# kontera-technologies/redis-bloomfilter

Hardware: AMD Instinct MI355X
Metric: keys/sec (insert, include?) per GPU and whole node; % of HBM random-access roofline (higher is better)
Workload: dtype u32

## Files before the change

redis-bloomfilter_amd/csrc/bf_binned.hip:

```cpp
#include "bf_device.h"

#include <algorithm>
#include <cmath>
#include <cstdlib>

using namespace bfdev;

namespace {
__device__ __forceinline__ void stage_store(uint32_t* p, uint32_t v) { __builtin_nontemporal_store(v, p); }
}

namespace {

constexpr int kTile = 1024;
constexpr int kStageVec = 16384 / 16;
constexpr uint32_t kMaxSup = 256;
constexpr uint32_t kMaxOwners = 256;
constexpr uint32_t kChunkBuckets = 512;
constexpr uint32_t kMaxRel = 9;
constexpr uint32_t kMaxBlocks = 512;
constexpr uint32_t kMaxFrontBlocks = 16384;
constexpr uint32_t kGroupBlocks = 64;
constexpr uint32_t kTileProbes = 12288;
constexpr int kSlots = 12;
constexpr int kWideSlots = 16;
constexpr uint32_t kTwoKeys = 6;
constexpr uint32_t kMaxTilesPerBlock = 16;
constexpr uint32_t kBlockProbes = 8192;
constexpr int kChunkPerLane = kBlockProbes / kTile;
constexpr uint32_t kRunsPerPass = 1024;
constexpr uint32_t kMidBuckets = 128;
constexpr uint32_t kMidParts = 2;
constexpr uint32_t kApplyLanes = 1024;
constexpr uint32_t kPipeLanes = 1024;

__device__ __forceinline__ uint32_t block_excl_scan(uint32_t v, uint32_t* s_w, uint32_t* total) {
    const uint32_t lane = threadIdx.x & 63u, wid = threadIdx.x >> 6, nw = blockDim.x >> 6;
    const uint32_t x = wave_incl_scan(v);
    if (lane == 63u) s_w[wid] = x;
    __syncthreads();
    if (wid == 0) {
        const uint32_t s = wave_incl_scan(lane < nw ? s_w[lane] : 0u);
        if (lane < nw) s_w[lane] = s;
    }
    __syncthreads();
    const uint32_t r = (wid ? s_w[wid - 1] : 0u) + x - v;
    if (total) *total = s_w[nw - 1];
    __syncthreads();
    return r;
}

template <bool KEYS, int SLOTS, bool DIG = false>
__device__ __forceinline__ void bin_front_body(BfGeom g, const uint8_t* __restrict__ keys16,
                                                          const uint64_t* __restrict__ offsets, uint64_t bias,
                                                          uint64_t n, uint32_t tile_keys, uint32_t tiles_per_block,
                                                          uint32_t sup_log2, uint32_t nsup,
                                                          uint32_t* __restrict__ level1,
                                                          uint32_t* __restrict__ level1_key,
                                                          uint16_t* __restrict__ stab, uint32_t* __restrict__ gcnt,
                                                          uint8_t* __restrict__ out8) {
    __shared__ uint64_t s_off[kTile + 1];
    __shared__ uint4 s_stage[kStageVec + kStageSlackVec];
    __shared__ uint32_t s_cnt[kMaxSup], s_lbase[kMaxSup], s_gcnt[kMaxSup];
    __shared__ uint32_t s_w[16];
    __shared__ uint32_t s_sorted[kTile * SLOTS];
    __shared__ uint32_t s_key[KEYS ? kTile * SLOTS : 1];
    const uint32_t t = threadIdx.x;
    if (t < kMaxSup) {
        s_cnt[t] = 0;
        s_gcnt[t] = 0;
    }
    __syncthreads();
    const uint32_t k = g.k;
    const uint32_t kpl = tile_keys / kTile;
    const uint64_t smask = (1ull << sup_log2) - 1ull;
    const uint64_t ntiles = (n + tile_keys - 1) / tile_keys;
    const uint64_t tb0 = (uint64_t)blockIdx.x * tiles_per_block;
    const uint64_t tb1 = (tb0 + tiles_per_block < ntiles) ? tb0 + tiles_per_block : ntiles;
    for (uint64_t tile = tb0; tile < tb1; ++tile) {
        const uint64_t key0 = tile * tile_keys;
        const uint32_t tk = (uint32_t)((n - key0) < (uint64_t)tile_keys ? (n - key0) : tile_keys);
        uint4 H0 = make_uint4(0, 0, 0, 0), H1 = make_uint4(0, 0, 0, 0);
        if constexpr (DIG) {
            const uint4* dig = reinterpret_cast<const uint4*>(keys16);
            if (t < tk) H0 = dig[key0 + t];
            if (kTile + t < tk) H1 = dig[key0 + kTile + t];
        } else {
            for_key_tile<kTile, kStageVec>(keys16, offsets, bias, key0, tk < (uint32_t)kTile ? tk : kTile, s_off,
                                           s_stage, g.key_status, [&](auto staged, uint32_t, const uint32_t* src, uint32_t s, uint32_t L) {
                uint32_t H[5];
                sha1_any<decltype(staged)::value>(src, s, L, H);
                H0 = make_uint4(H[0], H[1], H[2], H[3]);
            });
            if (tk > (uint32_t)kTile) {
                for_key_tile<kTile, kStageVec>(keys16, offsets, bias, key0 + kTile, tk - kTile, s_off, s_stage,
                    g.key_status, [&](auto staged, uint32_t, const uint32_t* src, uint32_t s, uint32_t L) {
                        uint32_t H[5];
                        sha1_any<decltype(staged)::value>(src, s, L, H);
                        H1 = make_uint4(H[0], H[1], H[2], H[3]);
                    });
            }
        }
        const bool live0 = t < tk;
        const bool live1 = kpl == 2 && kTile + t < tk;
        if constexpr (KEYS) {
            if (live0) out8[key0 + t] = 1;
            if (live1) out8[key0 + kTile + t] = 1;
        }
        uint32_t tag[SLOTS], loc[SLOTS];
#pragma unroll
        for (int q = 0; q < SLOTS; ++q) {
            const bool second = kpl == 2 && q >= (int)kTwoKeys;
            const uint32_t i = second ? (uint32_t)q - kTwoKeys : (uint32_t)q;
            const bool live = i < k && (second ? live1 : live0);
            tag[q] = 0xFFFFFFFFu;
            loc[q] = 0;
            if (live) {
                const uint4 H = second ? H1 : H0;
                const uint64_t o = probe_offset(g, H.x, H.y, H.z, H.w, i);
                const uint32_t sb = (uint32_t)(o >> sup_log2);
                tag[q] = (sb << 16) | atomicAdd(s_cnt + sb, 1u);
                loc[q] = (uint32_t)(o & smask);
            }
        }
        __syncthreads();
        const uint32_t c = t < kMaxSup ? s_cnt[t] : 0u;
        const uint32_t ex = block_excl_scan(c, s_w, nullptr);
        if (t <= nsup) stab[(uint64_t)t * ntiles + tile] = (uint16_t)ex;
        if (t < kMaxSup) {
            s_lbase[t] = ex;
            s_gcnt[t] += c;
            s_cnt[t] = 0;
        }
        __syncthreads();
#pragma unroll
        for (int q = 0; q < SLOTS; ++q) {
            if (tag[q] != 0xFFFFFFFFu) {
                const uint32_t d = s_lbase[tag[q] >> 16] + (tag[q] & 0xFFFFu);
                s_sorted[d] = loc[q];
                if constexpr (KEYS) {
                    const bool second = kpl == 2 && q >= (int)kTwoKeys;
                    s_key[d] = (uint32_t)(key0 + (second ? kTile + t : t));
                }
            }
        }
        __syncthreads();
        const uint64_t seg = key0 * k;
        const uint32_t tp = tk * k;
        for (uint32_t j = t; j < tp; j += kTile) {
            stage_store(level1 + seg + j, s_sorted[j]);
            if constexpr (KEYS) level1_key[seg + j] = s_key[j];
        }
    }
    if (t < nsup) gcnt[(uint64_t)blockIdx.x * nsup + t] = s_gcnt[t];
}

template <bool DIG>
__global__ __launch_bounds__(kTile) __attribute__((amdgpu_waves_per_eu(8, 8)))
void bin_front_kernel(BfGeom g, const uint8_t* __restrict__ keys16, const uint64_t* __restrict__ offsets,
                      uint64_t bias, uint64_t n, uint32_t tile_keys, uint32_t tiles_per_block, uint32_t sup_log2,
                      uint32_t nsup, uint32_t* __restrict__ level1, uint32_t* __restrict__ level1_key,
                      uint16_t* __restrict__ stab, uint32_t* __restrict__ gcnt, uint8_t* __restrict__ out8) {
    bin_front_body<false, kSlots, DIG>(g, keys16, offsets, bias, n, tile_keys, tiles_per_block, sup_log2, nsup,
                                       level1, level1_key, stab, gcnt, out8);
}

template <bool KEYS, bool DIG = false>
__global__ __launch_bounds__(kTile) void bin_front_wide_kernel(BfGeom g, const uint8_t* __restrict__ keys16,
                                                               const uint64_t* __restrict__ offsets, uint64_t bias,
                                                               uint64_t n, uint32_t tile_keys,
                                                               uint32_t tiles_per_block, uint32_t sup_log2,
                                                               uint32_t nsup, uint32_t* __restrict__ level1,
                                                               uint32_t* __restrict__ level1_key,
                                                               uint16_t* __restrict__ stab, uint32_t* __restrict__ gcnt,
                                                               uint8_t* __restrict__ out8) {
    bin_front_body<KEYS, kWideSlots, DIG>(g, keys16, offsets, bias, n, tile_keys, tiles_per_block, sup_log2, nsup,
                                          level1, level1_key, stab, gcnt, out8);
}

__global__ __launch_bounds__(kTile) __attribute__((amdgpu_waves_per_eu(8, 8)))
void bin_front_wide_dig_kernel(BfGeom g, const uint8_t* __restrict__ keys16, const uint64_t* __restrict__ offsets,
                               uint64_t bias, uint64_t n, uint32_t tile_keys, uint32_t tiles_per_block,
                               uint32_t sup_log2, uint32_t nsup, uint32_t* __restrict__ level1,
                               uint32_t* __restrict__ level1_key, uint16_t* __restrict__ stab,
                               uint32_t* __restrict__ gcnt, uint8_t* __restrict__ out8) {
    bin_front_body<false, kWideSlots, true>(g, keys16, offsets, bias, n, tile_keys, tiles_per_block, sup_log2, nsup,
                                            level1, level1_key, stab, gcnt, out8);
}

__global__ __launch_bounds__(kTile)
void bin_front_keys_kernel(BfGeom g, const uint8_t* __restrict__ keys16, const uint64_t* __restrict__ offsets,
                           uint64_t bias, uint64_t n, uint32_t tile_keys, uint32_t tiles_per_block, uint32_t sup_log2,
                           uint32_t nsup, uint32_t* __restrict__ level1, uint32_t* __restrict__ level1_key,
                           uint16_t* __restrict__ stab, uint32_t* __restrict__ gcnt, uint8_t* __restrict__ out8) {
    bin_front_body<true, kSlots>(g, keys16, offsets, bias, n, tile_keys, tiles_per_block, sup_log2, nsup, level1,
                                 level1_key, stab, gcnt, out8);
}

template <typename Off, bool KEYS>
__device__ __forceinline__ void bin_front_offsets_body(const Off* __restrict__ local, uint64_t count,
                                                       uint32_t tiles_per_block, uint32_t sup_log2, uint32_t nsup,
                                                       uint32_t* __restrict__ level1,
                                                       uint32_t* __restrict__ level1_key,
                                                       uint16_t* __restrict__ stab, uint32_t* __restrict__ gcnt,
                                                       uint64_t bias, const unsigned long long* __restrict__ wcounts,
                                                       uint32_t wstride, uint64_t wcap, uint64_t limit,
                                                       uint8_t* __restrict__ oob_out) {
    __shared__ uint32_t s_cnt[kMaxSup], s_lbase[kMaxSup], s_gcnt[kMaxSup];
    __shared__ uint32_t s_w[16];
    __shared__ uint32_t s_sorted[kTileProbes];
    __shared__ uint16_t s_key[KEYS ? kTileProbes : 1];
    const uint32_t t = threadIdx.x;
    if (t < kMaxSup) {
        s_cnt[t] = 0;
        s_gcnt[t] = 0;
    }
    __syncthreads();
    const uint64_t smask = (1ull << sup_log2) - 1ull;
    const uint64_t ntiles = (count + kTileProbes - 1) / kTileProbes;
    const bool vec_ok = (reinterpret_cast<uintptr_t>(local) & 15u) == 0;
    static_assert(kTileProbes == kTile * kSlots, "a tile is kSlots entries per lane");
    const uint64_t tb0 = (uint64_t)blockIdx.x * tiles_per_block;
    const uint64_t tb1 = (tb0 + tiles_per_block < ntiles) ? tb0 + tiles_per_block : ntiles;
    for (uint64_t tile = tb0; tile < tb1; ++tile) {
        const uint64_t p0 = tile * kTileProbes;
        uint32_t tp = (uint32_t)((count - p0) < (uint64_t)kTileProbes ? (count - p0) : kTileProbes);
        if (wcounts) {
            const uint64_t w = p0 / wcap, i0 = p0 - w * wcap;
            uint64_t live = wcounts[w * wstride];
            if (live > wcap) live = 0;
            tp = live > i0 ? (uint32_t)(live - i0 < (uint64_t)tp ? live - i0 : tp) : 0u;
        }
        uint32_t tag[kSlots], loc[kSlots];
        Off ent[kSlots];
        const uint32_t j0 = t * (uint32_t)kSlots;
        if (vec_ok && j0 + kSlots <= tp) {
            constexpr int kNV = kSlots * (int)sizeof(Off) / 16;
            const uint4* src = reinterpret_cast<const uint4*>(local + p0 + j0);
            uint4 vb[kNV];
#pragma unroll
            for (int v = 0; v < kNV; ++v) vb[v] = src[v];
            __builtin_memcpy(ent, vb, sizeof(ent));
        } else {
#pragma unroll
            for (int q = 0; q < kSlots; ++q) ent[q] = j0 + q < tp ? local[p0 + j0 + q] : (Off)0;
        }
#pragma unroll
        for (int q = 0; q < kSlots; ++q) {
            const uint32_t j = j0 + (uint32_t)q;
            tag[q] = 0xFFFFFFFFu;
            loc[q] = 0;
            if (j < tp) {
                const uint64_t o = (uint64_t)ent[q] + bias;
                if (o < limit) {
                    const uint32_t sb = (uint32_t)(o >> sup_log2);
                    tag[q] = (sb << 16) | atomicAdd(s_cnt + sb, 1u);
                    loc[q] = (uint32_t)(o & smask);
                } else if (oob_out) {
                    oob_out[p0 + j] = 0;
                }
            }
        }
        __syncthreads();
        const uint32_t c = t < kMaxSup ? s_cnt[t] : 0u;
        const uint32_t ex = block_excl_scan(c, s_w, nullptr);
        if (t <= nsup) stab[(uint64_t)t * ntiles + tile] = (uint16_t)ex;
        if (t < kMaxSup) {
            s_lbase[t] = ex;
            s_gcnt[t] += c;
            s_cnt[t] = 0;
        }
        __syncthreads();
#pragma unroll
        for (int q = 0; q < kSlots; ++q)
            if (tag[q] != 0xFFFFFFFFu) {
                const uint32_t d = s_lbase[tag[q] >> 16] + (tag[q] & 0xFFFFu);
                s_sorted[d] = loc[q];
                if constexpr (KEYS) s_key[d] = (uint16_t)(t * (uint32_t)kSlots + (uint32_t)q);
            }
        __syncthreads();
        for (uint32_t j = t; j < tp; j += kTile) {
            level1[p0 + j] = s_sorted[j];
            if constexpr (KEYS) level1_key[p0 + j] = (uint32_t)p0 + s_key[j];
        }
    }
    if (t < nsup) gcnt[(uint64_t)blockIdx.x * nsup + t] = s_gcnt[t];
}

template <typename Off>
__global__ __launch_bounds__(kTile) __attribute__((amdgpu_waves_per_eu(8, 8)))
void bin_front_offsets_kernel(const Off* __restrict__ local, uint64_t count, uint32_t tiles_per_block,
                              uint32_t sup_log2, uint32_t nsup, uint32_t* __restrict__ level1,
                              uint16_t* __restrict__ stab, uint32_t* __restrict__ gcnt, uint64_t bias,
                              const unsigned long long* __restrict__ wcounts, uint32_t wstride, uint64_t wcap,
                              uint64_t limit) {
    bin_front_offsets_body<Off, false>(local, count, tiles_per_block, sup_log2, nsup, level1, nullptr, stab, gcnt,
                                       bias, wcounts, wstride, wcap, limit, nullptr);
}

template <typename Off>
__global__ __launch_bounds__(kTile) __attribute__((amdgpu_waves_per_eu(8, 8)))
void bin_front_offsets_keys_kernel(const Off* __restrict__ local, uint64_t count,
                                                                       uint32_t tiles_per_block, uint32_t sup_log2,
                                                                       uint32_t nsup, uint32_t* __restrict__ level1,
                                                                       uint32_t* __restrict__ level1_key,
                                                                       uint16_t* __restrict__ stab,
                                                                       uint32_t* __restrict__ gcnt, uint64_t bias,
                                                                       const unsigned long long* __restrict__ wcounts,
                                                                       uint32_t wstride, uint64_t wcap, uint64_t limit,
                                                                       uint8_t* __restrict__ out8) {
    bin_front_offsets_body<Off, true>(local, count, tiles_per_block, sup_log2, nsup, level1, level1_key, stab, gcnt,
                                      bias, wcounts, wstride, wcap, limit, out8);
}

__global__ __launch_bounds__(kMaxBlocks) void bin_group_sum_kernel(const uint32_t* __restrict__ gcnt,
                                                                   uint32_t nblocks, uint32_t nsup, uint32_t nq,
                                                                   uint32_t* __restrict__ gsum) {
    const uint32_t sb = blockIdx.x;
    for (uint32_t w = threadIdx.x; w < nq * kGroupBlocks; w += kMaxBlocks) {
        uint32_t v = w < nblocks ? gcnt[(uint64_t)w * nsup + sb] : 0u;
#pragma unroll
        for (int off = 32; off > 0; off >>= 1) v += (uint32_t)__shfl_xor((int)v, off);
        if ((w & 63u) == 0) gsum[sb * nq + w / kGroupBlocks] = v;
    }
}

constexpr uint32_t kScanPer = 4;
constexpr uint32_t kScanWindows = 1024 * kScanPer;
constexpr uint32_t kLocalScanPer = 4;
constexpr uint32_t kMaxGroups = 1024 * kLocalScanPer;
constexpr uint32_t kMaxWindows = kMaxSup * kMaxGroups;
__global__ __launch_bounds__(1024) void bin_group_scan_kernel(const uint32_t* __restrict__ gsum, uint32_t N,
                                                              uint32_t* __restrict__ base,
                                                              uint32_t* __restrict__ cb_base,
                                                              uint32_t* __restrict__ cb_window,
                                                              uint32_t* __restrict__ cb_start, uint32_t nq,
                                                              unsigned long long* __restrict__ totals) {
    __shared__ uint32_t s_w[16];
    __shared__ uint32_t s_cb[kScanWindows + 1];
    const uint32_t t = threadIdx.x;
    uint32_t v[kScanPer], cv[kScanPer], sum = 0, csum = 0;
#pragma unroll
    for (uint32_t e = 0; e < kScanPer; ++e) {
        const uint32_t w = kScanPer * t + e;
        v[e] = w < N ? gsum[w] : 0u;
        cv[e] = (v[e] + kBlockProbes - 1) / kBlockProbes;
        sum += v[e];
        csum += cv[e];
    }
    uint32_t total, ctotal;
    uint32_t ex = block_excl_scan(sum, s_w, &total);
    uint32_t cex = block_excl_scan(csum, s_w, &ctotal);
// ... 271 lines not shown
                if constexpr (CHUNK)
                    reinterpret_cast<uint32_t*>(cg.dir + (uint64_t)t * cg.dir_bytes)[tile] =
                        (gb + oc <= wcap) ? (uint32_t)gb : 0xFFFFFFFFu;
            }
            if constexpr (CHUNK) {
                const uint32_t S1 = cg.S + 1u;
                for (uint32_t e = t; e < P * S1; e += kTile) {
                    const uint32_t w = e / S1, sb = e - w * S1;
                    const uint32_t b0 = (w * cg.S) << sub_log2, b1 = (w * cg.S + sb) << sub_log2;
                    const uint32_t v = (b1 < NB ? s_lbase[b1] : tk * k) - s_lbase[b0];
                    reinterpret_cast<uint16_t*>(cg.dir + (uint64_t)w * cg.dir_bytes + 4 * cg.tiles)
                        [(uint64_t)sb * cg.tiles + tile] = (uint16_t)v;
                }
            }
        }
#pragma unroll
        for (int q = 0; q < SLOTS; ++q) {
            if (tag[q] != 0xFFFFFFFFu) {
                const uint32_t d = s_lbase[tag[q] >> 16] + (tag[q] & 0xFFFFu);
                s_lo[d] = lo[q];
                if constexpr (WIDE) s_hi[d] = hi[q];
                if constexpr (SLOT) {
                    const bool second = kpl == 2 && q >= (int)kTwoKeys;
                    s_key[d] = (uint16_t)(second ? kTile + t : t);
                }
            }
        }
        __syncthreads();
        const uint64_t seg = key0 * k;
        const uint32_t tp = tk * k;
        if constexpr (WIN) {
            uint32_t o = run_of(s_obase, P, t < tp ? t : 0u);
            for (uint32_t j = t; j < tp; j += kTile) {
                while (o + 1u < P && s_obase[o + 1u] <= j) ++o;
                const unsigned long long gb = s_gbase[o];
                if (gb != ~0ull) {
                    const uint64_t d = gb + (j - s_obase[o]);
                    static_cast<uint32_t*>(wsend)[d] = s_lo[j];
                    if constexpr (SLOT) {
                        if constexpr (CHUNK) reinterpret_cast<uint16_t*>(wslot)[d] = s_key[j];
                        else wslot[d] = (uint32_t)key0 + s_key[j];
                    }
                }
            }
            __syncthreads();
        } else {
            for (uint32_t j = t; j < tp; j += kTile) {
                lo1[seg + j] = s_lo[j];
                if constexpr (WIDE) hi1[seg + j] = s_hi[j];
                if constexpr (SLOT) key1[seg + j] = (uint32_t)key0 + s_key[j];
            }
            if constexpr (SLOT) __syncthreads();
        }
    }
    if constexpr (!WIN)
        if (t < P) gcnt[(uint64_t)blockIdx.x * P + t] = s_gcnt[t];
}

#define BF_ROUTE_FRONT_ARGS                                                                                     \
    BfGeom g, const uint8_t* __restrict__ keys16, const uint64_t* __restrict__ offsets, uint64_t bias, uint64_t n, \
        uint32_t tile_keys, uint32_t tiles_per_block, uint32_t P, uint32_t* __restrict__ lo1,                   \
        uint8_t* __restrict__ hi1, uint32_t* __restrict__ key1, uint16_t* __restrict__ stab,                     \
        uint32_t* __restrict__ gcnt, uint64_t wcap, unsigned long long* __restrict__ wcounts,                 \
        void* __restrict__ wsend, uint32_t* __restrict__ wslot, uint32_t nh
#define BF_ROUTE_FRONT_PASS \
    g, keys16, offsets, bias, n, tile_keys, tiles_per_block, P, lo1, hi1, key1, stab, gcnt, wcap, wcounts, wsend, wslot, nh
template <bool WIDE, bool SLOT, int SLOTS, bool WIN, bool CHUNK = false, bool DIG = false>
__global__ __launch_bounds__(kTile) void route_front_kernel(BF_ROUTE_FRONT_ARGS, BfChunks cg) {
    route_front_body<WIDE, SLOT, SLOTS, WIN, CHUNK, DIG>(BF_ROUTE_FRONT_PASS, cg);
}
template <bool SLOT, bool WIN, bool CHUNK = false, bool DIG = false>
__global__ __launch_bounds__(kTile) __attribute__((amdgpu_waves_per_eu(8, 8)))
void route_front32_kernel(BF_ROUTE_FRONT_ARGS, BfChunks cg) {
    route_front_body<false, SLOT, kSlots, WIN, CHUNK, DIG>(BF_ROUTE_FRONT_PASS, cg);
}
#undef BF_ROUTE_FRONT_PASS
#undef BF_ROUTE_FRONT_ARGS

template <bool SLOT, int SLOTS, bool HASH = false>
__global__ __launch_bounds__(kTile) __attribute__((amdgpu_waves_per_eu(8, 8)))
void route_chunks_idx_kernel(BfGeom g, const uint8_t* __restrict__ keys16, const uint64_t* __restrict__ offsets,
                             uint64_t bias, uint64_t n, uint32_t tile_keys,
                             uint32_t tiles_per_block, uint32_t P, uint64_t wcap,
                             unsigned long long* __restrict__ wcounts, uint32_t* __restrict__ wsend,
                             uint16_t* __restrict__ wslot, uint32_t nh, BfChunks cg) {
    static_assert(SLOTS <= 16 && kTile * SLOTS <= 65536, "a probe index is 4 bits, a sort slot 16");
    constexpr uint32_t NB = kChunkBuckets;
    constexpr uint32_t kOffVec = (8 * (kTile + 1) + 15) / 16;
    static_assert(!HASH || (SLOTS > kSlots && (kOffVec + kStageVec + kStageSlackVec) * 16 <= kTile * SLOTS * 2),
                  "the key stage fits the index buffer (one key per lane)");
    __shared__ uint4 s_idx4[kTile * SLOTS * 2 / 16];
    uint16_t* s_idx = reinterpret_cast<uint16_t*>(s_idx4);
    __shared__ uint4 s_dig[SLOTS > kSlots ? kTile : 2 * kTile];
    const uint4* dig = reinterpret_cast<const uint4*>(keys16);
    __shared__ uint32_t s_cnt[NB], s_lbase[NB];
    __shared__ uint32_t s_w[16];
    __shared__ unsigned long long s_gbase[kMaxOwners];
    __shared__ uint32_t s_obase[kMaxOwners];
    const uint32_t sub_log2 = cg.sub2, wS = cg.S;
    const uint32_t t = threadIdx.x;
    if (t < NB) s_cnt[t] = 0;
    __syncthreads();
    const uint32_t k = g.k;
    const uint32_t kpl = tile_keys / kTile;
    const uint64_t ntiles = (n + tile_keys - 1) / tile_keys;
    const uint64_t tb0 = (uint64_t)blockIdx.x * tiles_per_block;
    const uint64_t tb1 = (tb0 + tiles_per_block < ntiles) ? tb0 + tiles_per_block : ntiles;
    for (uint64_t tile = tb0; tile < tb1; ++tile) {
        const uint64_t key0 = tile * tile_keys;
        const uint32_t tk = (uint32_t)((n - key0) < (uint64_t)tile_keys ? (n - key0) : tile_keys);
        const bool live0 = t < tk;
        const bool live1 = kpl == 2 && kTile + t < tk;
        uint4 H0 = make_uint4(0, 0, 0, 0), H1 = make_uint4(0, 0, 0, 0);
        if constexpr (HASH) {
            for_key_tile<kTile, kStageVec>(keys16, offsets, bias, key0, tk, reinterpret_cast<uint64_t*>(s_idx4),
                                           s_idx4 + kOffVec, g.key_status,
                [&](auto staged, uint32_t, const uint32_t* src, uint32_t s0, uint32_t L) {
                    uint32_t H[5];
                    sha1_any<decltype(staged)::value>(src, s0, L, H);
                    H0 = make_uint4(H[0], H[1], H[2], H[3]);
                });
        } else {
            if (live0) H0 = dig[key0 + t];
            if (live1) H1 = dig[key0 + kTile + t];
        }
        s_dig[t] = H0;
        if (kpl == 2) s_dig[kTile + t] = H1;
        uint32_t tag[SLOTS];
        auto probes = [&](auto kplc) {
            constexpr uint32_t KPL = decltype(kplc)::value;
#pragma unroll
            for (int q = 0; q < SLOTS; ++q) {
                const bool second = KPL == 2 && q >= (int)kTwoKeys;
                const uint32_t i = second ? (uint32_t)q - kTwoKeys : (uint32_t)q;
                tag[q] = 0xFFFFFFFFu;
                if (i < k && (second ? live1 : live0)) {
                    const uint4 H = second ? H1 : H0;
                    uint32_t owner;
                    uint64_t local;
                    owner_local(g, probe_offset(g, H.x, H.y, H.z, H.w, i), owner, local);
                    const uint32_t lo = (uint32_t)local;
                    uint32_t sb = lo >> cg.sup_log2;
                    if (sb >= cg.S) sb = cg.S - 1u;
                    const uint32_t wb = (owner * nh + (uint32_t)(local >> 32)) * cg.S + sb;
                    const uint32_t bkt = (wb << sub_log2) | (lo & ((1u << sub_log2) - 1u));
                    tag[q] = (bkt << 16) | atomicAdd(s_cnt + bkt, 1u);
                }
            }
        };
        if (kpl == 2) probes(std::integral_constant<uint32_t, 2>{});
        else probes(std::integral_constant<uint32_t, 1>{});
        __syncthreads();
        const uint32_t c = t < NB ? s_cnt[t] : 0u;
        const uint32_t ex = block_excl_scan(c, s_w, nullptr);
        if (t < NB) {
            s_lbase[t] = ex;
            s_cnt[t] = 0;
        }
        __syncthreads();
        if (t < P) {
            const uint32_t lo_b = (t * wS) << sub_log2, hi_b = ((t + 1) * wS) << sub_log2;
            const uint32_t ob = s_lbase[lo_b], oc = (hi_b < NB ? s_lbase[hi_b] : tk * k) - ob;
            unsigned long long gb = 0;
            if (oc) {
                uint8_t* dw = cg.dir + (uint64_t)t * cg.dir_bytes;
                const unsigned long long x = atomicAdd(
                    reinterpret_cast<unsigned long long*>(dw + bf_chunk_dir_claim_offset(cg, cg.tiles)),
                    (1ull << kClaimRankShift) | (unsigned long long)oc);
                gb = x & ((1ull << kClaimRankShift) - 1ull);
                reinterpret_cast<uint16_t*>(dw + bf_chunk_dir_rank_offset(cg, cg.tiles))[x >> kClaimRankShift] =
                    (uint16_t)(tile + 1u);
                atomicAdd(wcounts + t, (unsigned long long)oc);
            }
            s_gbase[t] = (gb + oc <= wcap) ? (unsigned long long)t * wcap + gb : ~0ull;
            s_obase[t] = ob;
            reinterpret_cast<uint32_t*>(cg.dir + (uint64_t)t * cg.dir_bytes)[tile] =
                (gb + oc <= wcap) ? (uint32_t)gb : 0xFFFFFFFFu;
        }
        {
            const uint32_t S1 = cg.S + 1u;
            for (uint32_t e = t; e < P * S1; e += kTile) {
                const uint32_t w = e / S1, sb = e - w * S1;
                const uint32_t b0 = (w * cg.S) << sub_log2, b1 = (w * cg.S + sb) << sub_log2;
                const uint32_t v = (b1 < NB ? s_lbase[b1] : tk * k) - s_lbase[b0];
                reinterpret_cast<uint16_t*>(cg.dir + (uint64_t)w * cg.dir_bytes + 4 * cg.tiles)
                    [(uint64_t)sb * cg.tiles + tile] = (uint16_t)v;
            }
        }
        auto place = [&](auto kplc) {
            constexpr uint32_t KPL = decltype(kplc)::value;
#pragma unroll
            for (int q = 0; q < SLOTS; ++q)
                if (tag[q] != 0xFFFFFFFFu) {
                    const bool second = KPL == 2 && q >= (int)kTwoKeys;
                    const uint32_t i = second ? (uint32_t)q - kTwoKeys : (uint32_t)q;
                    s_idx[s_lbase[tag[q] >> 16] + (tag[q] & 0xFFFFu)] = (uint16_t)(((second ? kTile + t : t) << 4) | i);
                }
        };
        if (kpl == 2) place(std::integral_constant<uint32_t, 2>{});
        else place(std::integral_constant<uint32_t, 1>{});
        __syncthreads();
        const uint32_t tp = tk * k;
        uint32_t o = run_of(s_obase, P, t < tp ? t : 0u);
        for (uint32_t j = t; j < tp; j += kTile) {
            while (o + 1u < P && s_obase[o + 1u] <= j) ++o;
            const unsigned long long gb = s_gbase[o];
            if (gb == ~0ull) continue;
            const uint32_t x = s_idx[j], key = x >> 4;
            const uint4 H = s_dig[key];
            uint32_t owner;
            uint64_t local;
            owner_local(g, probe_offset(g, H.x, H.y, H.z, H.w, x & 15u), owner, local);
            const uint64_t d = gb + (j - s_obase[o]);
            wsend[d] = (uint32_t)local;
            if constexpr (SLOT) wslot[d] = (uint16_t)key;
        }
        __syncthreads();
    }
}

template <bool WIDE, bool SLOT>
__global__ __launch_bounds__(kTile) void route_gather_kernel(const uint32_t* __restrict__ lo1,
                                                             const uint8_t* __restrict__ hi1,
                                                             const uint32_t* __restrict__ key1,
                                                             const uint16_t* __restrict__ stab, uint64_t ntiles,
                                                             uint32_t tile_probes, uint32_t tiles_per_group,
                                                             uint32_t nowners, uint32_t nq,
                                                             const uint32_t* __restrict__ base,
                                                             const uint32_t* __restrict__ cb_base,
                                                             const uint32_t* __restrict__ cb_window,
                                                             void* __restrict__ send, uint32_t* __restrict__ slot) {
    __shared__ uint32_t s_pre[kRunsPerPass], s_gst[kRunsPerPass];
    __shared__ uint32_t s_w[16];
    const uint32_t t = threadIdx.x, b = blockIdx.x;
    if (b >= cb_base[nowners * nq]) return;
    const uint32_t w = cb_window[b];
    const uint32_t owner = w / nq, q = w - owner * nq;
    const uint32_t wbase = base[w];
    const uint32_t E = base[w + 1] - wbase;
    const uint32_t f0 = (b - cb_base[w]) * kBlockProbes;
    const uint32_t f_end = (E - f0 < kBlockProbes) ? E : f0 + kBlockProbes;
    const uint64_t tlo = (uint64_t)q * tiles_per_group;
    const uint64_t thi = (tlo + tiles_per_group < ntiles) ? tlo + tiles_per_group : ntiles;
    const uint32_t nt = (uint32_t)(thi - tlo);
    uint32_t len = 0, st = 0;
    if (t < nt) {
        const uint32_t a = stab[(uint64_t)owner * ntiles + tlo + t];
        len = stab[(uint64_t)(owner + 1) * ntiles + tlo + t] - a;
        st = (uint32_t)((tlo + t) * tile_probes) + a;
    }
    const uint32_t ex = block_excl_scan(len, s_w, nullptr);
    if (t < nt) {
        s_pre[t] = ex;
        s_gst[t] = st;
    }
    __syncthreads();
    const uint32_t fw = f0 + (t >> 6) * (64u * kChunkPerLane);
    uint32_t i = run_of(s_pre, nt, fw < f_end ? fw : f_end - 1);
#pragma unroll
    for (int u = 0; u < kChunkPerLane; ++u) {
        const uint32_t f = fw + u * 64 + (t & 63u);
        if (f < f_end) {
            while (i + 1 < nt && s_pre[i + 1] <= f) ++i;
            const uint32_t idx = s_gst[i] + (f - s_pre[i]);
            if constexpr (WIDE)
                static_cast<uint64_t*>(send)[wbase + f] = ((uint64_t)hi1[idx] << 32) | lo1[idx];
            else
                static_cast<uint32_t*>(send)[wbase + f] = lo1[idx];
            if constexpr (SLOT) slot[wbase + f] = key1[idx];
        }
    }
}

__device__ __forceinline__ uint32_t mid_superbin(uint32_t nsup, uint32_t nq, bool grouped, uint32_t* q,
                                                 uint32_t* part) {
    if (!grouped) {
        const uint32_t w = blockIdx.x / kMidParts;
        *part = blockIdx.x - w * kMidParts;
        *q = w % nq;
        return w / nq;
    }
    const uint32_t wpsb = nq * kMidParts, xi = blockIdx.x >> 3;
    const uint32_t i = xi / wpsb, wq = xi - i * wpsb;
    *q = wq / kMidParts;
    *part = wq - *q * kMidParts;
    return (blockIdx.x & 7u) + 8u * i;
}
__host__ __device__ inline bool mid_grouped(uint32_t nsup) { return nsup >= 64; }
uint32_t mid_grid(uint32_t nsup, uint32_t nq) {
    return mid_grouped(nsup) ? 8u * ((nsup + 7u) / 8u) * nq * kMidParts : nsup * nq * kMidParts;
}

template <bool KEYS>
__global__ __launch_bounds__(kTile) __attribute__((amdgpu_waves_per_eu(8, 8))) void bin_mid_kernel(const uint32_t* __restrict__ level1,
                                                        const uint32_t* __restrict__ level1_key,
                                                        const uint16_t* __restrict__ stab, uint64_t ntiles,
                                                        uint32_t tile_probes, uint32_t tiles_per_group,
                                                        uint32_t nsup, uint32_t nq, uint32_t region_log2,
                                                        uint32_t rel_log2, const uint32_t* __restrict__ base,
                                                        const uint32_t* __restrict__ cb_base, uint64_t max_chunks,
                                                        uint16_t* __restrict__ tabs, uint32_t* __restrict__ level2,
                                                        uint32_t* __restrict__ level2_key) {
    __shared__ uint32_t s_pre[kRunsPerPass], s_gst[kRunsPerPass];
    __shared__ uint32_t s_cnt[1u << kMaxRel];
    __shared__ uint32_t s_w[16];
    __shared__ uint32_t s_sorted[kBlockProbes];
    __shared__ uint32_t s_key[KEYS ? kBlockProbes : 1];
    const uint32_t t = threadIdx.x;
    uint32_t w_q, w_part;
    const uint32_t sb = mid_superbin(nsup, nq, mid_grouped(nsup), &w_q, &w_part);
    if (sb >= nsup) return;
    const uint32_t q = w_q, part = w_part;
    const uint32_t w = sb * nq + q;
    const uint32_t wbase = base[w];
    const uint32_t E = base[w + 1] - wbase;
    const uint32_t nblk = (E + kBlockProbes - 1) / kBlockProbes;
    const uint32_t c_lo = (uint32_t)((uint64_t)nblk * part / kMidParts);
    const uint32_t c_hi = (uint32_t)((uint64_t)nblk * (part + 1) / kMidParts);
    if (c_lo >= c_hi) return;
    const uint32_t b0 = cb_base[w];
    const uint32_t R = 1u << rel_log2;
    const uint32_t rmask = (1u << region_log2) - 1u;
    uint32_t sub = 0;
    while ((R << sub) < kMidBuckets) ++sub;
    const uint32_t NB = R << sub, smask_b = (1u << sub) - 1u;
    const uint64_t tlo = (uint64_t)q * tiles_per_group;
    const uint64_t thi = (tlo + tiles_per_group < ntiles) ? tlo + tiles_per_group : ntiles;
    const uint32_t nt = (uint32_t)(thi - tlo);
    uint32_t len = 0, st = 0;
    if (t < nt) {
        const uint32_t a = stab[(uint64_t)sb * ntiles + tlo + t];
        len = stab[(uint64_t)(sb + 1) * ntiles + tlo + t] - a;
        st = (uint32_t)((tlo + t) * tile_probes) + a;
    }
    const uint32_t ex = block_excl_scan(len, s_w, nullptr);
    if (t < nt) {
        s_pre[t] = ex;
        s_gst[t] = st;
    }
    __syncthreads();
    auto load = [&](uint32_t f0, uint32_t* lv, uint32_t* kv) {
        const uint32_t fw = f0 + (t >> 6) * (64u * kChunkPerLane);
        uint32_t i = run_of(s_pre, nt, fw < E ? fw : E - 1);
#pragma unroll
        for (int u = 0; u < kChunkPerLane; ++u) {
            const uint32_t f = fw + u * 64 + (t & 63u);
            lv[u] = 0xFFFFFFFFu;
            kv[u] = 0;
            if (f < E) {
                while (i + 1 < nt && s_pre[i + 1] <= f) ++i;
                const uint32_t idx = s_gst[i] + (f - s_pre[i]);
                lv[u] = level1[idx];
                if constexpr (KEYS) kv[u] = level1_key[idx];
            }
        }
    };
    uint32_t lv[kChunkPerLane], kv[kChunkPerLane];
    load(c_lo * kBlockProbes, lv, kv);
    for (uint32_t c = c_lo; c < c_hi; ++c) {
        const uint32_t f0 = c * kBlockProbes;
        const uint32_t f1 = (E - f0 < kBlockProbes) ? E : f0 + kBlockProbes;
        if (t < NB) s_cnt[t] = 0;
        __syncthreads();
        uint32_t tag[kChunkPerLane];
#pragma unroll
        for (int u = 0; u < kChunkPerLane; ++u) {
            tag[u] = 0xFFFFFFFFu;
            if (lv[u] != 0xFFFFFFFFu) {
                const uint32_t bk = ((lv[u] >> region_log2) << sub) | (lv[u] & smask_b);
                tag[u] = (bk << 16) | atomicAdd(s_cnt + bk, 1u);
            }
        }
        uint32_t nlv[kChunkPerLane], nkv[kChunkPerLane];
        if (c + 1 < c_hi) load(f0 + kBlockProbes, nlv, nkv);
        __syncthreads();
        const uint32_t cn = t < NB ? s_cnt[t] : 0u;
        const uint32_t cex = block_excl_scan(cn, s_w, nullptr);
        if (!(t & smask_b) && (t >> sub) <= R)
            tabs[(uint64_t)(t >> sub) * max_chunks + b0 + c] = (uint16_t)cex;
        if (t < NB) s_cnt[t] = cex;
        __syncthreads();
#pragma unroll
        for (int u = 0; u < kChunkPerLane; ++u) {
            if (tag[u] != 0xFFFFFFFFu) {
                const uint32_t d = s_cnt[tag[u] >> 16] + (tag[u] & 0xFFFFu);
                s_sorted[d] = lv[u] & rmask;
                if constexpr (KEYS) s_key[d] = kv[u];
            }
        }
        __syncthreads();
        const uint32_t out0 = wbase + f0;
        for (uint32_t j = t; j < f1 - f0; j += kTile) {
            stage_store(level2 + out0 + j, s_sorted[j]);
            if constexpr (KEYS) level2_key[out0 + j] = s_key[j];
        }
        if (c + 1 < c_hi) {
#pragma unroll
            for (int u = 0; u < kChunkPerLane; ++u) {
                lv[u] = nlv[u];
                kv[u] = nkv[u];
            }
        }
    }
}

template <int kLoads, typename Visit>
__device__ __forceinline__ void for_region_probes(const uint32_t* __restrict__ cb_base,
                                                  const uint32_t* __restrict__ cb_start,
                                                  const uint16_t* __restrict__ tabs, uint64_t max_chunks, uint32_t r,
                                                  uint32_t nq, uint32_t rel_log2, uint32_t* s_pre, uint32_t* s_gst,
                                                  uint32_t* s_w, Visit&& visit) {
    const uint32_t R = 1u << rel_log2;
    const uint32_t sb = r >> rel_log2, rl = r & (R - 1u);
    const uint32_t t = threadIdx.x, lanes = blockDim.x;
    const uint32_t bb0 = cb_base[sb * nq], bb1 = cb_base[(sb + 1) * nq];
    const uint32_t pass = lanes < kRunsPerPass ? lanes : kRunsPerPass;
    for (uint32_t p0 = bb0; p0 < bb1; p0 += pass) {
        const uint32_t nt = (bb1 - p0 < pass) ? bb1 - p0 : pass;
        uint32_t len = 0, st = 0;
        if (t < nt) {
            const uint32_t a = tabs[(uint64_t)rl * max_chunks + p0 + t];
            len = tabs[(uint64_t)(rl + 1) * max_chunks + p0 + t] - a;
            st = cb_start[p0 + t] + a;
        }
        uint32_t E;
        const uint32_t ex = block_excl_scan(len, s_w, &E);
        if (t < nt) {
            s_pre[t] = ex;
            s_gst[t] = st;
        }
        __syncthreads();
        const uint32_t span = kLoads * 64u, lane = t & 63u;
        for (uint32_t fb = 0; fb < E; fb += span * (lanes >> 6)) {
            const uint32_t fw = fb + (t >> 6) * span;
            uint32_t idx[kLoads];
#pragma unroll
            for (int c = 0; c < kLoads; ++c) idx[c] = 0xFFFFFFFFu;
            if (fw < E) {
                uint32_t i0 = 0;
                for (uint32_t b = 0; b < nt; b += 64u) {
                    const uint32_t j = b + lane;
                    const uint32_t c = (uint32_t)__popcll(__ballot(j < nt && s_pre[j] <= fw));
                    if (c) i0 = b + c - 1u;
                    if (c < 64u) break;
                }
                const uint32_t fend = E - fw < span ? E : fw + span;
                uint32_t ic[kLoads];
#pragma unroll
                for (int c = 0; c < kLoads; ++c) ic[c] = i0;
                for (uint32_t i = i0 + 1u; i < nt; ++i) {
                    const uint32_t B = __builtin_amdgcn_readfirstlane(s_pre[i]);
                    if (B >= fend) break;
#pragma unroll
                    for (int c = 0; c < kLoads; ++c) ic[c] += (fw + c * 64u + lane >= B) ? 1u : 0u;
                }
#pragma unroll
                for (int c = 0; c < kLoads; ++c) {
                    const uint32_t f = fw + c * 64u + lane;
                    if (f < E) idx[c] = s_gst[ic[c]] + (f - s_pre[ic[c]]);
                }
            }
            visit(idx);
        }
        __syncthreads();
    }
}

typedef uint32_t apply_u32x4 __attribute__((ext_vector_type(4)));
__device__ __forceinline__ uint4 apply_load(const uint4* p) { return *p; }
__device__ __forceinline__ void apply_store(uint4* p, uint4 v) {
    const apply_u32x4 x = {v.x, v.y, v.z, v.w};
    __builtin_nontemporal_store(x, reinterpret_cast<apply_u32x4*>(p));
}

__device__ __forceinline__ uint32_t apply_region(uint32_t b, uint32_t nb, uint32_t xg) {
    if (xg <= 1) return b;
    const uint32_t span = 8u * xg, full = nb - nb % span;
    if (b >= full) return b;
    const uint32_t w = b % span;
    return b - w + (w & 7u) * xg + (w >> 3);
}

template <uint32_t RLOG2, uint32_t LANES, int LOADS = 8>
__global__ __launch_bounds__(LANES) void bin_apply_kernel(uint32_t* __restrict__ bits, uint64_t nwords,
                                                          const uint32_t* __restrict__ level2,
                                                          const uint32_t* __restrict__ cb_base,
                                                          const uint32_t* __restrict__ cb_start,
                                                          const uint16_t* __restrict__ tabs, uint64_t max_chunks,
                                                          uint32_t nq, uint32_t rel_log2, uint32_t dense,
                                                          uint32_t* __restrict__ any_flag,
                                                          uint8_t* __restrict__ dirty, uint32_t store_fresh,
                                                          uint32_t xg) {
    constexpr uint32_t kVec = 1u << (RLOG2 - 7);
    constexpr uint32_t kPer = kVec / LANES;
    constexpr int kLoads = LOADS;
    static_assert(kPer * LANES == kVec, "region must tile the workgroup");
    __shared__ uint4 s_mask4[kVec];
    __shared__ uint32_t s_pre[kRunsPerPass], s_gst[kRunsPerPass], s_w[16];
    uint32_t* s_mask = reinterpret_cast<uint32_t*>(s_mask4);
    const uint32_t t = threadIdx.x;
    const uint32_t r = apply_region(blockIdx.x, gridDim.x, xg);
    const uint64_t v0 = (uint64_t)r * kVec;
    const uint64_t nvec = nwords / 4;
    uint4* gv = reinterpret_cast<uint4*>(bits);
    uint4 old[kPer];
#pragma unroll
    for (uint32_t c = 0; c < kPer; ++c) {
        const uint32_t v = c * LANES + t;
        old[c] = make_uint4(0, 0, 0, 0);
        if (dense && v0 + v < nvec) old[c] = apply_load(gv + v0 + v);
    }
    for (uint32_t v = t; v < kVec; v += LANES) s_mask4[v] = make_uint4(0, 0, 0, 0);
    __syncthreads();
    for_region_probes<kLoads>(cb_base, cb_start, tabs, max_chunks, r, nq, rel_log2, s_pre, s_gst, s_w,
        [&](const uint32_t* idx) {
            uint32_t l[kLoads];
#pragma unroll
            for (int c = 0; c < kLoads; ++c) l[c] = idx[c] != 0xFFFFFFFFu ? level2[idx[c]] : 0xFFFFFFFFu;
#pragma unroll
            for (int c = 0; c < kLoads; ++c)
                if (l[c] != 0xFFFFFFFFu) atomicOr(s_mask + (l[c] >> 5), 1u << ((l[c] ^ 7u) & 31u));
        });
    uint4 msk[kPer];
#pragma unroll
    for (uint32_t c = 0; c < kPer; ++c) {
        const uint32_t v = c * LANES + t;
        msk[c] = s_mask4[v];
        if (!dense && v0 + v < nvec && (msk[c].x | msk[c].y | msk[c].z | msk[c].w)) old[c] = apply_load(gv + v0 + v);
    }
    uint32_t fresh = 0;
#pragma unroll
    for (uint32_t c = 0; c < kPer; ++c) {
        const uint32_t v = c * LANES + t;
        const uint32_t fr = (msk[c].x & ~old[c].x) | (msk[c].y & ~old[c].y) | (msk[c].z & ~old[c].z) |
                            (msk[c].w & ~old[c].w);
        fresh |= fr;
        if (v0 + v >= nvec) continue;
        bool st;
        if (dense == 2) st = true;
        else if (store_fresh) st = fr != 0u;
        else st = (msk[c].x | msk[c].y | msk[c].z | msk[c].w) != 0u;
        if (st)
            apply_store(gv + v0 + v, make_uint4(old[c].x | msk[c].x, old[c].y | msk[c].y, old[c].z | msk[c].z, old[c].w | msk[c].w));
        if (dirty && fr) dirty[((v0 + v) * 128) >> kDirtyShiftBits] = 1;
    }
    if (any_flag) report_any_new(any_flag, fresh != 0);
}

constexpr int kWaitVm0 = 0x0F70;
template <uint32_t RLOG2, uint32_t LANES, int LOADS = 8>
__global__ __launch_bounds__(LANES) __attribute__((amdgpu_waves_per_eu(4, 4))) void bin_apply_pipe_kernel(uint32_t* __restrict__ bits, uint64_t nwords,
                                                               uint32_t nbins, const uint32_t* __restrict__ level2,
                                                               const uint32_t* __restrict__ cb_base,
                                                               const uint32_t* __restrict__ cb_start,
                                                               const uint16_t* __restrict__ tabs, uint64_t max_chunks,
                                                               uint32_t nq, uint32_t rel_log2, uint32_t dense,
                                                               uint32_t* __restrict__ any_flag,
                                                               uint8_t* __restrict__ dirty, uint32_t store_fresh) {
    constexpr uint32_t kVec = 1u << (RLOG2 - 7);
    constexpr uint32_t kPer = kVec / LANES;
    constexpr int kLoads = LOADS;
    constexpr uint32_t kPass = LANES < kRunsPerPass ? LANES : kRunsPerPass;
    static_assert(kPer * LANES == kVec, "region must tile the workgroup");
    __shared__ uint4 s_mask4[kVec];
    __shared__ uint32_t s_pre[2][kPass], s_gst[2][kPass], s_w[16];
    uint32_t* s_mask = reinterpret_cast<uint32_t*>(s_mask4);
    const uint32_t t = threadIdx.x;
    const uint32_t R = 1u << rel_log2;
    const uint64_t nvec = nwords / 4;
    uint4* gv = reinterpret_cast<uint4*>(bits);
    const uint32_t G = gridDim.x;
    const uint32_t span = kLoads * 64u, step = span * (LANES >> 6);
    if (blockIdx.x >= nbins) return;
    const uint32_t last = blockIdx.x + (nbins - 1 - blockIdx.x) / G * G;
    auto clampr = [&](uint32_t q) { return q < last ? q : last; };

    struct Tab { uint32_t a, b, cs; };
    auto load_tab = [&](uint32_t q) {
        const uint32_t sb = q >> rel_log2, rl = q & (R - 1u);
        const uint32_t bb0 = cb_base[sb * nq], bb1 = cb_base[(sb + 1) * nq];
        const uint32_t nt = bb1 - bb0;
        const uint64_t j = nt ? bb0 + (t < nt ? t : nt - 1u) : 0u;
        Tab x;
        x.a = tabs[(uint64_t)rl * max_chunks + j];
        x.b = tabs[(uint64_t)(rl + 1) * max_chunks + j];
        x.cs = cb_start[j];
        return x;
    };
    auto scan = [&](uint32_t nt, uint32_t len, uint32_t st, uint32_t bi) {
        uint32_t E;
        const uint32_t ex = block_excl_scan(t < nt ? len : 0u, s_w, &E);
        if (t < nt) {
            s_pre[bi][t] = ex;
            s_gst[bi][t] = st;
        }
        __syncthreads();
        return E;
    };
    auto pass_nt = [&](uint32_t q) {
        const uint32_t sb = q >> rel_log2;
        const uint32_t n = cb_base[(sb + 1) * nq] - cb_base[sb * nq];
        return n < kPass ? n : kPass;
    };
    auto load_l2 = [&](uint32_t bi, uint32_t nt, uint32_t E, uint32_t fb, uint32_t* l) {
        const uint32_t fw = fb + (t >> 6) * span;
        uint32_t i = (nt && fw < E) ? run_of(s_pre[bi], nt, fw) : 0u;
#pragma unroll
        for (int c = 0; c < kLoads; ++c) {
            const uint32_t f = fw + c * 64 + (t & 63u);
            uint32_t idx = 0;
            if (f < E) {
                while (i + 1 < nt && s_pre[bi][i + 1] <= f) ++i;
                idx = s_gst[bi][i] + (f - s_pre[bi][i]);
            }
            l[c] = level2[idx];
        }
    };
    auto mark = [&](const uint32_t* l, uint32_t E, uint32_t fb) {
        const uint32_t fw = fb + (t >> 6) * span;
#pragma unroll
        for (int c = 0; c < kLoads; ++c)
            if (fw + c * 64 + (t & 63u) < E) atomicOr(s_mask + (l[c] >> 5), 1u << ((l[c] ^ 7u) & 31u));
    };
    auto load_vecs = [&](uint32_t q, uint4* vo) {
        const uint64_t v0 = (uint64_t)q * kVec;
#pragma unroll
        for (uint32_t c = 0; c < kPer; ++c) {
            const uint64_t v = v0 + c * LANES + t;
            vo[c] = apply_load(gv + (v < nvec ? v : nvec - 1));
        }
    };

    uint32_t fresh = 0;
    auto region = [&](uint32_t r, uint32_t bi, uint32_t nt, uint32_t E, const uint4* cur, const uint32_t* lv,
                      const Tab& tn, uint4* nxt, uint32_t* nlv, Tab& tnn, uint32_t& ntn) {
        const uint32_t rn = clampr(r + G);
        ntn = pass_nt(rn);
        const uint32_t En = scan(ntn, tn.b - tn.a, tn.cs + tn.a, bi ^ 1u);
        tnn = load_tab(clampr(r + 2 * G));
        load_l2(bi ^ 1u, ntn, En, 0, nlv);
        load_vecs(rn, nxt);
        mark(lv, E, 0);
        for (uint32_t fb = step; fb < E; fb += step) {
            uint32_t l[kLoads];
            load_l2(bi, nt, E, fb, l);
            mark(l, E, fb);
            __builtin_amdgcn_s_waitcnt(kWaitVm0);
        }
        const uint32_t sb = r >> rel_log2, rl = r & (R - 1u);
        const uint32_t bb0 = cb_base[sb * nq], bb1 = cb_base[(sb + 1) * nq];
        for (uint32_t p0 = bb0 + kPass; p0 < bb1; p0 += kPass) {
            const uint32_t pn = (bb1 - p0 < kPass) ? bb1 - p0 : kPass;
            uint32_t len = 0, st = 0;
            if (t < pn) {
                const uint32_t a = tabs[(uint64_t)rl * max_chunks + p0 + t];
                len = tabs[(uint64_t)(rl + 1) * max_chunks + p0 + t] - a;
                st = cb_start[p0 + t] + a;
            }
            __syncthreads();
            const uint32_t Ep = scan(pn, len, st, bi);
            for (uint32_t fb = 0; fb < Ep; fb += step) {
                uint32_t l[kLoads];
                load_l2(bi, pn, Ep, fb, l);
                mark(l, Ep, fb);
            }
            __builtin_amdgcn_s_waitcnt(kWaitVm0);
        }
        __syncthreads();
        const uint64_t v0 = (uint64_t)r * kVec;
#pragma unroll
        for (uint32_t c = 0; c < kPer; ++c) {
            const uint32_t v = c * LANES + t;
            const uint4 m = s_mask4[v];
            s_mask4[v] = make_uint4(0, 0, 0, 0);
            if (v0 + v < nvec && (dense == 2 || (m.x | m.y | m.z | m.w))) {
                const uint32_t fr = (m.x & ~cur[c].x) | (m.y & ~cur[c].y) | (m.z & ~cur[c].z) | (m.w & ~cur[c].w);
                fresh |= fr;
                if (store_fresh && dense != 2 && !fr) continue;
                apply_store(gv + v0 + v, make_uint4(cur[c].x | m.x, cur[c].y | m.y, cur[c].z | m.z, cur[c].w | m.w));
                if (dirty && fr) dirty[((v0 + v) * 128) >> kDirtyShiftBits] = 1;
            }
        }
        return En;
    };

    uint32_t r = blockIdx.x;
    for (uint32_t v = t; v < kVec; v += LANES) s_mask4[v] = make_uint4(0, 0, 0, 0);
    uint4 bufA[kPer], bufB[kPer];
    uint32_t lA[kLoads], lB[kLoads];
    Tab tA, tB;
    uint32_t ntA, ntB, EA, EB;
    {
        const Tab t0 = load_tab(r);
        ntA = pass_nt(r);
        EA = scan(ntA, t0.b - t0.a, t0.cs + t0.a, 0u);
        tA = load_tab(clampr(r + G));
        load_l2(0u, ntA, EA, 0, lA);
// ... 2289 lines not shown
```

Before: 13.55 billion.

## Double-buffer mid-bin counters, narrow-wave scan, and vectorize level2 stores

In the keyless bin_mid_kernel path, the bucket counters are double-buffered so the per-chunk zeroing barrier goes away. The next buffer is cleared during the scan. The block-wide exclusive scan is replaced by a scan run only on the waves that cover the bucket count, using readlane so no extra LDS barrier rounds are needed. Output to level2 is realigned to 16 bytes and written with 4-wide nontemporal stores, with scalar head and tail stores. This adds alignment bookkeeping and extra LDS, and the narrow scan loops over earlier waves' counts serially.

```diff
diff --git a/redis-bloomfilter_amd/csrc/bf_binned.hip b/redis-bloomfilter_amd/csrc/bf_binned.hip
--- a/redis-bloomfilter_amd/csrc/bf_binned.hip
+++ b/redis-bloomfilter_amd/csrc/bf_binned.hip
@@ -8,6 +8,10 @@
 
 namespace {
 __device__ __forceinline__ void stage_store(uint32_t* p, uint32_t v) { __builtin_nontemporal_store(v, p); }
+typedef uint32_t stage_u32x4 __attribute__((ext_vector_type(4)));
+__device__ __forceinline__ void stage_store4(uint32_t* p, const uint32_t* lds) {
+    __builtin_nontemporal_store(*reinterpret_cast<const stage_u32x4*>(lds), reinterpret_cast<stage_u32x4*>(p));
+}
 }
 
 namespace {
@@ -48,6 +52,16 @@
     if (total) *total = s_w[nw - 1];
     __syncthreads();
     return r;
+}
+
+__device__ __forceinline__ uint32_t narrow_excl_scan(const uint32_t* cnt, uint32_t cap) {
+    const uint32_t t = threadIdx.x, lane = t & 63u, wid = t >> 6;
+    const uint32_t c = t < cap ? cnt[t] : 0u;
+    uint32_t below = 0;
+    for (uint32_t j = 0; j < wid; ++j) below += cnt[j * 64u + lane];
+    const uint32_t x = wave_incl_scan(c);
+    const uint32_t off = (uint32_t)__builtin_amdgcn_readlane((int)wave_incl_scan(below), 63);
+    return off + x - c;
 }
 
 template <bool KEYS, int SLOTS, bool DIG = false>
@@ -925,9 +939,9 @@
                                                         uint16_t* __restrict__ tabs, uint32_t* __restrict__ level2,
                                                         uint32_t* __restrict__ level2_key) {
     __shared__ uint32_t s_pre[kRunsPerPass], s_gst[kRunsPerPass];
-    __shared__ uint32_t s_cnt[1u << kMaxRel];
+    __shared__ uint32_t s_cnt2[KEYS ? 1 : 2][1u << kMaxRel], s_bases[KEYS ? 1 : 1u << kMaxRel];
     __shared__ uint32_t s_w[16];
-    __shared__ uint32_t s_sorted[kBlockProbes];
+    __shared__ __attribute__((aligned(16))) uint32_t s_sorted[kBlockProbes + 4];
     __shared__ uint32_t s_key[KEYS ? kBlockProbes : 1];
     const uint32_t t = threadIdx.x;
     uint32_t w_q, w_part;
@@ -961,6 +975,12 @@
         s_pre[t] = ex;
         s_gst[t] = st;
     }
+    if constexpr (!KEYS) {
+        if (t < (1u << kMaxRel)) {
+            s_cnt2[0][t] = 0;
+            s_cnt2[1][t] = 0;
+        }
+    }
     __syncthreads();
     auto load = [&](uint32_t f0, uint32_t* lv, uint32_t* kv) {
         const uint32_t fw = f0 + (t >> 6) * (64u * kChunkPerLane);
@@ -978,13 +998,20 @@
             }
         }
     };
+    const uint32_t scan_waves = (NB + 64u) >> 6;
+    uint32_t par = 0;
+    const uint32_t al = KEYS ? 0u : (uint32_t)(reinterpret_cast<uintptr_t>(level2 + wbase) >> 2) & 3u;
     uint32_t lv[kChunkPerLane], kv[kChunkPerLane];
     load(c_lo * kBlockProbes, lv, kv);
     for (uint32_t c = c_lo; c < c_hi; ++c) {
         const uint32_t f0 = c * kBlockProbes;
         const uint32_t f1 = (E - f0 < kBlockProbes) ? E : f0 + kBlockProbes;
-        if (t < NB) s_cnt[t] = 0;
-        __syncthreads();
+        uint32_t* const s_cnt = s_cnt2[par];
+        uint32_t* const s_base = KEYS ? s_cnt : s_bases;
+        if constexpr (KEYS) {
+            if (t < NB) s_cnt[t] = 0;
+            __syncthreads();
+        }
         uint32_t tag[kChunkPerLane];
 #pragma unroll
         for (int u = 0; u < kChunkPerLane; ++u) {
@@ -997,25 +1024,48 @@
         uint32_t nlv[kChunkPerLane], nkv[kChunkPerLane];
         if (c + 1 < c_hi) load(f0 + kBlockProbes, nlv, nkv);
         __syncthreads();
-        const uint32_t cn = t < NB ? s_cnt[t] : 0u;
-        const uint32_t cex = block_excl_scan(cn, s_w, nullptr);
-        if (!(t & smask_b) && (t >> sub) <= R)
-            tabs[(uint64_t)(t >> sub) * max_chunks + b0 + c] = (uint16_t)cex;
-        if (t < NB) s_cnt[t] = cex;
+        if constexpr (KEYS) {
+            const uint32_t cn = t < NB ? s_cnt[t] : 0u;
+            const uint32_t cex = block_excl_scan(cn, s_w, nullptr);
+            if (!(t & smask_b) && (t >> sub) <= R)
+                tabs[(uint64_t)(t >> sub) * max_chunks + b0 + c] = (uint16_t)cex;
+            if (t < NB) s_base[t] = cex;
+        } else {
+            if ((t >> 6) < scan_waves) {
+                const uint32_t cex = narrow_excl_scan(s_cnt, NB);
+                if (!(t & smask_b) && (t >> sub) <= R)
+                    tabs[(uint64_t)(t >> sub) * max_chunks + b0 + c] = (uint16_t)cex;
+                if (t < NB) {
+                    s_base[t] = cex;
+                    s_cnt2[par ^ 1u][t] = 0;
+                }
+            }
+            par ^= 1u;
+        }
         __syncthreads();
 #pragma unroll
         for (int u = 0; u < kChunkPerLane; ++u) {
             if (tag[u] != 0xFFFFFFFFu) {
-                const uint32_t d = s_cnt[tag[u] >> 16] + (tag[u] & 0xFFFFu);
-                s_sorted[d] = lv[u] & rmask;
+                const uint32_t d = s_base[tag[u] >> 16] + (tag[u] & 0xFFFFu);
+                s_sorted[al + d] = lv[u] & rmask;
                 if constexpr (KEYS) s_key[d] = kv[u];
             }
         }
         __syncthreads();
         const uint32_t out0 = wbase + f0;
-        for (uint32_t j = t; j < f1 - f0; j += kTile) {
-            stage_store(level2 + out0 + j, s_sorted[j]);
-            if constexpr (KEYS) level2_key[out0 + j] = s_key[j];
+        if constexpr (KEYS) {
+            for (uint32_t j = t; j < f1 - f0; j += kTile) {
+                stage_store(level2 + out0 + j, s_sorted[j]);
+                level2_key[out0 + j] = s_key[j];
+            }
+        } else {
+            uint32_t* const dst = level2 + out0 - al;
+            const uint32_t pe = al + (f1 - f0);
+            const uint32_t v0 = (al + 3u) & ~3u, he = v0 < pe ? v0 : pe;
+            const uint32_t v1 = pe & ~3u, ts = v1 > he ? v1 : he;
+            if (al + t < he) stage_store(dst + al + t, s_sorted[al + t]);
+            for (uint32_t j = v0 + 4u * t; j < v1; j += 4u * kTile) stage_store4(dst + j, s_sorted + j);
+            if (ts + t < pe) stage_store(dst + ts + t, s_sorted[ts + t]);
         }
         if (c + 1 < c_hi) {
 #pragma unroll
```

Result: no change. 13.47 billion (median of 2 runs) (-0.6%).
